# librosa/librosa

Hardware: AMD Instinct MI355X
Metric: STFT+mel frames/sec (n_fft=2048 hop=512) (higher is better)
Workload: dtype f32

## Files before the change

librosa_amd/csrc/lra_api.hip:

```cpp
#include <dlfcn.h>
#include <hip/hip_runtime.h>
#include <rocfft/rocfft.h>

#include <algorithm>
#include <atomic>
#include <chrono>
#include <cmath>
#include <cstdio>
#include <cstdlib>
#include <cstring>
#include <map>
#include <memory>
#include <mutex>
#include <string>
#include <thread>
#include <vector>

#include "../../include/librosa_amd.h"
#define LRA_FUSED_EXTERN
#include "lra_fused.h"
#include "lra_mel.h"
#include "lra_post.h"
#include "lra_pcen.h"
#include "lra_onset.h"
#include "lra_cqt.h"
#include "lra_hpss.h"
#include "lra_probe.h"
#include "lra_rng.h"
#include "lra_mixed_launch.h"
#include "lra_rhythm_launch.h"
#include "lra_beat_launch.h"
#include "lra_peaks_launch.h"
#include "lra_chroma_launch.h"

using namespace lra;

static thread_local std::string g_err;

static int fail(int code, const std::string& msg) {
    g_err = msg;
    return code;
}
#define LRA_HIP(expr)                                                                                        \
    do {                                                                                                     \
        hipError_t e__ = (expr);                                                                             \
        if (e__ != hipSuccess) return fail(LRA_EHIP, std::string(#expr) + ": " + hipGetErrorString(e__));    \
    } while (0)
#define LRA_FFT(expr)                                                                                        \
    do {                                                                                                     \
        rocfft_status s__ = (expr);                                                                          \
        if (s__ != rocfft_status_success) return fail(LRA_EROCFFT, std::string(#expr) + ": rocfft status " + std::to_string((int)s__)); \
    } while (0)
#define LRA_TRY(expr)              \
    do {                           \
        int rc__ = (expr);         \
        if (rc__ != LRA_OK) return rc__; \
    } while (0)

struct lra_ctx {
    int device = 0;
    hipStream_t own_stream = nullptr;
    hipStream_t stream = nullptr;
    int n_cu = 256;
    int opt_stft_iters = 0;
    int opt_istft_strip_groups = 0;
    int opt_variant = -1;
    int opt_autotune = 1;
    int opt_mel_runs = 1;
    int opt_mel_tile = 0;
    int opt_generic_mel = 0;
    int opt_lds_pad = 0;
    int opt_v2 = 1;
    int opt_istft16 = 0;
    int opt_placement_retry = 0;
    struct PlacedAlloc {
        size_t padded = 0;
        std::vector<hipMemGenericAllocationHandle_t> handles;
        bool plain = false;
    };
    std::map<void*, PlacedAlloc> placed;
    std::mutex placed_mu;
    std::vector<std::pair<void*, size_t>> placed_retired;
    size_t placed_va_spent = 0;
    static constexpr size_t kPlacedVaBudget = (size_t)4 << 40;
    double placed_best_gbps = 0.0;
    int opt_v3 = 1;
    int opt_mel_pc = 1;
    int opt_mel_many = 1;
    int opt_cqt_merge = 1;
    int opt_hpss_tile = 1;
    int opt_mixed_inv_pow2 = 1;
    int opt_mixed_pow2_mel = 1;
    int opt_ola4 = 1;
    int opt_mixed_irfft = 1;
    int opt_mixed = 1;
    int opt_direct = 1;
    int opt_xcd_remap = 1;
    unsigned int* d_flag = nullptr;
    std::map<std::pair<int, int>, std::pair<void*, void*>> cqt_tw;
    std::string name;
    struct HostPipe* pipe = nullptr;
    hipStream_t side_stream = nullptr;
    hipStream_t side_main = nullptr;
    static constexpr int kForkRing = 16;
    hipEvent_t fork_event[kForkRing] = {}, side_passed[kForkRing] = {};
    bool fork_used[kForkRing] = {};
    int fork_next = 0;
    static constexpr int kJoinRing = 8;
    hipEvent_t join_event[kJoinRing] = {}, main_passed[kJoinRing] = {};
    bool join_used[kJoinRing] = {};
    int join_next = 0;
    bool on_side = false, side_used = false;
    struct ResampleFft* rs_fft = nullptr;
    int opt_pipe_chunk_mb = 128;
    int opt_pipe_threads = 8;
};

// ... 146 lines not shown
    int* d_melr_addr = nullptr;
    int melr_zero = 0, melr_mid = 0, melr_pmax = 0;
    bool melr_ok = false;
    bool melr_many = false;
    void* d_melr2_w = nullptr;
    void* d_melr2_keep = nullptr;
    int* d_melr2_addr = nullptr;
    int melr2_zero = 0, melr2_mid = 0, melr2_pmax = 0;
    bool melr2_ok = false;
    int* d_run[2] = {nullptr, nullptr};
    int* d_segd[2] = {nullptr, nullptr};
    int nyq[2] = {0, 0};
    int n_pieces[2] = {0, 0};
};

struct lra_istft_plan {
    lra_ctx* ctx = nullptr;
    int n_fft = 0, hop = 0, center = 0, dtype = 0;
    bool pow2 = false;
    int logm = 0;
    void* d_win_scaled = nullptr;
    void* d_tw[kNumVariants] = {};
    int tuned_variant[4] = {-1, -1, -1, -1};
    void* d_twr = nullptr;
    FftPlanCache fft;
    Scratch spec, frames;
    Scratch norm;
    void* d_mtw = nullptr;
    void* d_mtwn = nullptr;
};

namespace {

static int resident_workgroups(const void* kern, int block, int lds) {
    static std::mutex mu;
    static std::map<std::pair<const void*, int>, int> cache;
    std::lock_guard<std::mutex> lk(mu);
    const auto key = std::make_pair(kern, lds);
    auto it = cache.find(key);
    if (it != cache.end()) return it->second;
    int per_cu = 0;
    if (lds > 65536) (void)hipFuncSetAttribute(kern, hipFuncAttributeMaxDynamicSharedMemorySize, lds);
    if (hipOccupancyMaxActiveBlocksPerMultiprocessor(&per_cu, kern, block, lds) != hipSuccess) per_cu = 0;
    (void)hipGetLastError();
    cache[key] = per_cu;
    return per_cu;
}

template <class T> struct StftLaunch {
    StftArgs<T> a;
    int mode = 0;
    long long batch = 0;
    int iters_opt = 0;
    int mel_tile_opt = 0;
    int n_cu = 256;
    void* out = nullptr;
    int lds_pad = 0;
    bool xcd_remap = true;
    bool use_v2 = true;
    bool use_direct = true;
    bool mel_v2 = false;
    bool mel_pc = false;
    bool mel_runs = true;
    const lra_mel_plan* mel = nullptr;
    hipStream_t stream = nullptr;
    hipError_t err = hipSuccess;

    template <class Cfg, int MODE> void launch(int shared_bytes) {
        static_assert(Cfg::P <= 4, "at most four Stockham passes are wired up");
        const int lds_probe_v1 = Cfg::FPB * stft_slot_bytes<Cfg>(MODE, a.n_mels, mel_tile_opt > 0 ? mel_tile_opt : 4) + shared_bytes + lds_pad;
        void (*kern)(StftArgs<T>, const T*, void*) = nullptr;
        bool direct = false;
        if constexpr (Cfg::PLAN == 0) {
        kern = stft_kernel<Cfg, MODE, POW_TWO, 0>;
        if (MODE != OUT_COMPLEX && a.power_mode == POW_ONE) kern = stft_kernel<Cfg, MODE, POW_ONE, 0>;
        if (MODE != OUT_COMPLEX && a.power_mode == POW_GENERAL) kern = stft_kernel<Cfg, MODE, POW_GENERAL, 0>;
        if constexpr (sizeof(T) == 4) {
            if (ring_rows_aligned<Cfg>(a.hop)) {
                kern = stft_kernel<Cfg, MODE, POW_TWO, 1>;
                if (MODE != OUT_COMPLEX && a.power_mode == POW_ONE) kern = stft_kernel<Cfg, MODE, POW_ONE, 1>;
                if (MODE != OUT_COMPLEX && a.power_mode == POW_GENERAL) kern = stft_kernel<Cfg, MODE, POW_GENERAL, 1>;
            }
        }
        if constexpr (MODE == OUT_COMPLEX || MODE == OUT_POWER) {
            if (a.hop >= Cfg::N && use_direct) {
                direct = true;
                kern = stft_kernel<Cfg, MODE, POW_TWO, 2>;
                if (MODE != OUT_COMPLEX && a.power_mode == POW_ONE) kern = stft_kernel<Cfg, MODE, POW_ONE, 2>;
                if (MODE != OUT_COMPLEX && a.power_mode == POW_GENERAL) kern = stft_kernel<Cfg, MODE, POW_GENERAL, 2>;
            }
        }
        if constexpr ((MODE == OUT_COMPLEX || MODE == OUT_POWER) && sizeof(T) == 4 && (Cfg::LOGM >= 12 || Cfg::LOGM == 7 || Cfg::LOGM == 8)) {
            const int hd = use_direct ? regring_hd<Cfg>(a.hop) : 0;
#define LRA_PICKR(RAM)                                                                                       \
    kern = stft_kernel<Cfg, MODE, POW_TWO, RAM>;                                                            \
    if (MODE != OUT_COMPLEX && a.power_mode == POW_ONE) kern = stft_kernel<Cfg, MODE, POW_ONE, RAM>;        \
    if (MODE != OUT_COMPLEX && a.power_mode == POW_GENERAL) kern = stft_kernel<Cfg, MODE, POW_GENERAL, RAM>;
            if (hd == 2) { direct = true; LRA_PICKR(3) } else if (hd == 4) { direct = true; LRA_PICKR(4) } else if (hd == 8) { direct = true; LRA_PICKR(5) } else if (hd == 16) { direct = true; LRA_PICKR(6) }
#undef LRA_PICKR
        }
        }
        bool v2 = false;
        if constexpr (v23_cfg_ok<Cfg>() && (MODE == OUT_COMPLEX || MODE == OUT_POWER || MODE == OUT_MELR)) {
            const int hd = (use_v2 && (MODE != OUT_MELR || mel_v2)) ? v2_hop_divisor<Cfg>(a.hop) : 0;
            if (hd) {
                v2 = true;
// ... 11 lines not shown
        if (iters <= 0) {
            const int per_cu = lds_probe <= 160 * 1024 ? resident_workgroups(reinterpret_cast<const void*>(kern), Cfg::NT, lds_probe) : 0;
            const long long conc = (long long)n_cu * (per_cu > 0 ? per_cu : 1);
            const int fpb = Cfg::FPB;
            int best_iters = 0;
            double best_fill = -1.0;
            for (int cand = 176; cand >= 24; --cand) {
                const int wgpc = (a.n_frames + fpb * cand - 1) / (fpb * cand);
                const int it = (a.n_frames + fpb * wgpc - 1) / (fpb * wgpc);
                const double rounds = (double)(batch * wgpc) / (double)conc;
                const double fill = (v2 && Cfg::TF == 64 && rounds <= 1.0 && rounds >= 0.6) ? 1.0 : rounds / std::ceil(rounds);
                if (fill > best_fill + 0.02) { best_fill = fill; best_iters = it; }
            }
            iters = best_iters;
            while (iters > 4 && batch * ((a.n_frames + fpb * iters - 1) / (fpb * iters)) < 2LL * n_cu) iters /= 2;
        }
        if (iters < 1) iters = 1;
        a.rot_uniform = 0;
        if (Cfg::FPB > 1 && Cfg::TF < 64 && ring_rows_aligned<Cfg>(a.hop)) {
            if (iters_opt <= 0 && iters >= 4) iters = (iters + 3) / 4 * 4;
            a.rot_uniform = iters % 4 == 0;
        }
        a.mel_tile = mel_tile_opt > 0 ? mel_tile_opt : 4;
        if (a.mel_tile > iters) a.mel_tile = iters;
        a.frames_per_wg = Cfg::FPB * iters;
        a.wg_per_clip = (a.n_frames + a.frames_per_wg - 1) / a.frames_per_wg;
        a.slot_bytes = v2 ? stft2_slot_bytes<Cfg>() : direct ? Cfg::FRAME_BYTES : stft_slot_bytes<Cfg>(MODE, a.n_mels, a.mel_tile);
        a.shared_off = Cfg::FPB * a.slot_bytes;
        const long long grid = batch * a.wg_per_clip;
        if (grid > 0x7ffffff0LL) { err = hipErrorInvalidConfiguration; return; }
        const int lds = Cfg::FPB * a.slot_bytes + shared_bytes + lds_pad;
        if (lds > 160 * 1024) { err = hipErrorInvalidValue; return; }
        if (lds > 65536) {
            err = hipFuncSetAttribute(reinterpret_cast<const void*>(kern), hipFuncAttributeMaxDynamicSharedMemorySize, lds);
            if (err != hipSuccess) return;
        }
        a.n_blocks = (int)grid;
        a.xcd_chunk = (xcd_remap && grid >= 64) ? (int)((grid + 7) / 8) : 0;
        const long long launch_grid = a.xcd_chunk ? 8LL * a.xcd_chunk : grid;
        hipLaunchKernelGGL(kern, dim3((unsigned)launch_grid), dim3(Cfg::NT), lds, stream, a, a.y, out);
        err = hipGetLastError();
    }

    template <class Cfg> void launch_pc(int hd) {
        using PL = PcLayout<Cfg>;
        void (*kern)(StftArgs<T>, const T*, void*) = nullptr;
#define LRA_PICKP(HD)                                                        \
    kern = stft_pc_kernel<Cfg, HD, POW_TWO>;                                 \
    if (a.power_mode == POW_ONE) kern = stft_pc_kernel<Cfg, HD, POW_ONE>;    \
    if (a.power_mode == POW_GENERAL) kern = stft_pc_kernel<Cfg, HD, POW_GENERAL>;
        if (hd == 4) { LRA_PICKP(4) } else { LRA_PICKP(8) }
#undef LRA_PICKP
        const int lds = PL::BYTES + lds_pad;
        constexpr int fpb = PL::NP;
        int iters = iters_opt;
        if (iters <= 0) {
            const int per_cu = resident_workgroups(reinterpret_cast<const void*>(kern), PL::NT, lds);
            const long long conc = (long long)n_cu * (per_cu > 0 ? per_cu : 1);
            int best_iters = 0;
            double best_fill = -1.0;
            for (int cand = 176; cand >= 24; --cand) {
                const int wgpc = (a.n_frames + fpb * cand - 1) / (fpb * cand);
                const int it = (a.n_frames + fpb * wgpc - 1) / (fpb * wgpc);
                const double rounds = (double)(batch * wgpc) / (double)conc;
                const double fill = (rounds <= 1.0 && rounds >= 0.6) ? 1.0 : rounds / std::ceil(rounds);
                if (fill > best_fill + 0.02) { best_fill = fill; best_iters = it; }
            }
            iters = best_iters;
            while (iters > 4 && batch * ((a.n_frames + fpb * iters - 1) / (fpb * iters)) < 2LL * n_cu) iters /= 2;
        }
        if (iters < 1) iters = 1;
        a.rot_uniform = 0;
        a.mel_tile = 1;
        a.frames_per_wg = fpb * iters;
        a.wg_per_clip = (a.n_frames + a.frames_per_wg - 1) / a.frames_per_wg;
        a.slot_bytes = PL::FRAME;
        a.shared_off = 0;
        const long long grid = batch * a.wg_per_clip;
        if (grid > 0x7ffffff0LL) { err = hipErrorInvalidConfiguration; return; }
        a.n_blocks = (int)grid;
        a.xcd_chunk = (xcd_remap && grid >= 64) ? (int)((grid + 7) / 8) : 0;
        const long long launch_grid = a.xcd_chunk ? 8LL * a.xcd_chunk : grid;
        hipLaunchKernelGGL(kern, dim3((unsigned)launch_grid), dim3(PL::NT), lds, stream, a, a.y, out);
        err = hipGetLastError();
    }

    template <class Cfg> void operator()() {
        if constexpr (Cfg::REV) {
            err = hipErrorInvalidValue;
            return;
        } else if constexpr (Cfg::PLAN == 1) {
            if (!use_v2 || v2_hop_divisor<Cfg>(a.hop) == 0) { err = hipErrorInvalidValue; return; }
            if (mode == OUT_COMPLEX) launch<Cfg, OUT_COMPLEX>(0);
            else if (mode == OUT_POWER) launch<Cfg, OUT_POWER>(0);
            else if (mode == OUT_MEL2 && mel_pc && mel && mel->melr2_ok && mel_runs) {
                if constexpr (pc_cfg_ok<Cfg>()) {
                    const int hd_pc = v2_hop_divisor<Cfg>(a.hop);
                    if (!pc_bank_ok<Cfg>(a.n_mels, mel->melr2_pmax) || !pc_fits_budget<Cfg>(hd_pc, a.power_mode)) { err = hipErrorInvalidValue; return; }
                    a.melr_w = (const T*)mel->d_melr2_w;
                    a.melr_keep = (const T*)mel->d_melr2_keep;
                    a.melr_addr = mel->d_melr2_addr;
                    a.melr_zero = mel->melr2_zero;
                    a.melr_mid = mel->melr2_mid;
                    a.melr_pmax = mel->melr2_pmax;
                    launch_pc<Cfg>(hd_pc);
                } else err = hipErrorInvalidValue;
            } else err = hipErrorInvalidValue;
        } else {
            run<Cfg>();
        }
    }
    template <class Cfg> void run() {
        if (mode == OUT_MEL2) {
            using MC = typename MelCfgOf<Cfg>::type;
            if constexpr (pc_cfg_ok<Cfg>()) {
                const int hd_pc = v2_hop_divisor<Cfg>(a.hop);
                if (mel_pc && mel && mel->melr2_ok && mel_runs && use_v2 && pc_bank_ok<Cfg>(a.n_mels, mel->melr2_pmax) && pc_fits_budget<Cfg>(hd_pc, a.power_mode)) {
                    a.melr_w = (const T*)mel->d_melr2_w;
                    a.melr_keep = (const T*)mel->d_melr2_keep;
                    a.melr_addr = mel->d_melr2_addr;
                    a.melr_zero = mel->melr2_zero;
                    a.melr_mid = mel->melr2_mid;
                    a.melr_pmax = mel->melr2_pmax;
                    launch_pc<Cfg>(hd_pc);
                    return;
                }
            }
            if constexpr (v2_cfg_ok<MC>()) {
                if (mel && mel->melr2_ok && mel_runs && use_v2 && melr_fits<MC>() && v2_hop_divisor<MC>(a.hop) > 0) {
                    const int shared_r = melr_shared_bytes<MC>(a.n_mels, mel->melr2_pmax);
                    if (MC::FPB * stft2_slot_bytes<MC>() + shared_r <= 160 * 1024) {
                        a.melr_w = (const T*)mel->d_melr2_w;
                        a.melr_keep = (const T*)mel->d_melr2_keep;
                        a.melr_addr = mel->d_melr2_addr;
                        a.melr_zero = mel->melr2_zero;
// ... 492 lines not shown
}

template <class T>
int stft_run(lra_stft_plan* p, int mode, const void* y, int64_t batch, int64_t n, int64_t y_stride, double power, lra_mel_plan* mel, void* out, int64_t row_pitch = 0) {
    LRA_BIND(p->ctx);
    int64_t n_frames = 0;
    LRA_TRY(lra_stft_num_frames(p, n, &n_frames));
    if (batch <= 0) return LRA_OK;
    if (!y || !out) return fail(LRA_EINVAL, "null data pointer");
    if (y_stride < n) return fail(LRA_EINVAL, "y_stride smaller than n");
    if (n_frames > 0x7fffffffLL / 4) return fail(LRA_EINVAL, "too many frames per clip");
    lra_ctx* ctx = p->ctx;
    const int bins = p->n_fft / 2 + 1;
    if (row_pitch <= 0) row_pitch = bins;
    if (row_pitch != bins && (!p->pow2 || row_pitch < bins || (mode != OUT_COMPLEX && mode != OUT_POWER)))
        return fail(LRA_EINVAL, "a row pitch other than n_bins is served by the fused power-of-two kernels only (complex / power results), and must be at least n_bins");
    if (mode == OUT_MEL) {
        if (!mel) return fail(LRA_EINVAL, "null mel plan");
        if (mel->n_bins != bins) return fail(LRA_EINVAL, "mel basis has " + std::to_string(mel->n_bins) + " bins, stft has " + std::to_string(bins));
        if (mel->dtype != p->dtype) return fail(LRA_EINVAL, "mel plan dtype differs from stft plan dtype");
    }
    const bool pow2_mel_mixed = p->pow2 && mode == OUT_MEL && p->d_mtw && ctx->opt_mixed && ctx->opt_mixed_pow2_mel && row_pitch == bins && mel &&
                                mel->n_mels >= (p->n_fft >= 256 ? 56 : 40);
    if (p->pow2 && !pow2_mel_mixed) {
        StftLaunch<T> L;
        L.a = StftArgs<T>();
        L.a.y = (const T*)y;
        L.a.y_stride = y_stride;
        L.a.n = n;
        L.a.n_frames = (int)n_frames;
        L.a.row_pitch = row_pitch;
        L.a.hop = p->hop;
        L.a.pad = p->center ? p->n_fft / 2 : 0;
        L.a.pad_mode = p->pad_mode;
        L.a.win = (const T*)p->d_win;
        L.a.twr = (const cx<T>*)p->d_twr;
        L.out = out;
        L.a.power_mode = power_mode_of(power);
        L.a.power = (T)power;
        if (mel) {
            L.a.mel_c0 = mel->d_c0;
            L.a.mel_len = mel->d_len;
            L.a.mel_off = mel->d_off;
            L.a.mel_val = (const T*)mel->d_val;
            L.a.n_mels = mel->n_mels;
            L.a.mel_wAB = (const T*)mel->d_wAB;
            L.mel = mel;
        }
        L.a.nonfinite_flag = ctx->d_flag;
        L.mode = (mode == OUT_MEL && mel && mel->two_slope && !ctx->opt_generic_mel) ? OUT_MEL2 : mode;
        L.batch = batch;
        L.stream = ctx->stream;
        L.iters_opt = ctx->opt_stft_iters;
        L.n_cu = ctx->n_cu;
        L.mel_tile_opt = ctx->opt_mel_tile;
        L.lds_pad = ctx->opt_lds_pad;
        L.xcd_remap = ctx->opt_xcd_remap != 0;
        L.use_v2 = ctx->opt_v2 != 0;
        L.mel_pc = ctx->opt_mel_pc != 0;
        L.use_direct = ctx->opt_direct != 0;
        L.mel_runs = ctx->opt_mel_runs != 0;
        int variant = ctx->opt_variant >= 0 ? ctx->opt_variant : 0;
        auto launch = [&](int v) -> int {
            StftLaunch<T> Lv = L;
            Lv.a.tw = (const cx<T>*)p->d_tw[v];
            if (!dispatch_logm<T>(p->logm, v, Lv)) return fail(LRA_EINVAL, "unsupported power-of-two size");
            if (Lv.err != hipSuccess) return fail(LRA_EHIP, std::string("stft kernel launch: ") + hipGetErrorString(Lv.err));
            return LRA_OK;
        };
        bool v2_applies = false;
        if constexpr (sizeof(T) == 4)
            v2_applies = ctx->opt_v2 && (L.mode == OUT_COMPLEX || L.mode == OUT_POWER) && p->logm == 10 && v2_hop_divisor<typename CfgSel<float, 10, 0>::type>(p->hop) > 0;
        if (ctx->opt_variant < 0 && ctx->opt_autotune && sizeof(T) == 4 && p->logm == 10 && !v2_applies) {
            int& tuned = p->tuned_variant[L.mode & 3];
            if (tuned < 0 && batch * n_frames >= 65536) LRA_TRY(autotune_variant(ctx, launch, &tuned));
            if (tuned >= 0) variant = tuned;
        }
        bool pc_g = false;
        if constexpr (sizeof(T) == 4) {
            using C6 = typename CfgSel<float, 10, 6>::type;
            if (L.mode == OUT_MEL2 && ctx->opt_mel_pc == 2 && p->logm == 10 && mel && mel->melr2_ok && ctx->opt_mel_runs && ctx->opt_v2 && (ctx->opt_variant < 0 || ctx->opt_variant == 6))
                pc_g = pc_bank_ok<C6>(mel->n_mels, mel->melr2_pmax) && pc_fits_budget<C6>(v2_hop_divisor<C6>(p->hop), power_mode_of(power));
        }
        if ((v2_applies && (ctx->opt_v3 == 2 || (ctx->opt_v3 == 1 && L.mode == OUT_COMPLEX)) && (ctx->opt_variant < 0 || ctx->opt_variant == 6)) || pc_g) variant = 6;
        else if (variant == 6) variant = 0;
        return launch(variant);
    }
    if (p->d_mtw && ctx->opt_mixed) {
        mixed::Args<T> a = mixed::Args<T>();
        a.y = (const T*)y;
        a.y_stride = y_stride;
        a.n = n;
        a.n_frames = (int)n_frames;
        a.hop = p->hop;
        a.pad = p->center ? p->n_fft / 2 : 0;
        a.pad_mode = p->pad_mode;
        a.win = (const T*)(p->pow2 ? p->d_win_full : p->d_win);
        a.tw_m = (const mixed::cpx<T>*)p->d_mtw;
        a.tw_n = (const mixed::cpx<T>*)p->d_mtwn;
        a.power_mode = power_mode_of(power);
        a.power = (T)power;
        const int F = mixed::frames_per_group_of(p->n_fft, (int)sizeof(T));
        a.groups_per_clip = (int)((n_frames + F - 1) / F);
        int mm = mixed::MIXED_COMPLEX;
        if (mode == OUT_COMPLEX) {
            a.D = (mixed::cpx<T>*)out;
// ... 607 lines not shown
                LRA_HIP(hipStreamCreateWithFlags(&ctx->side_stream, hipStreamNonBlocking));
        }
        const int slot = ctx->fork_next;
        ctx->fork_next = (slot + 1) % lra_ctx::kForkRing;
        if (!ctx->fork_event[slot]) LRA_HIP(hipEventCreateWithFlags(&ctx->fork_event[slot], hipEventDisableTiming));
        if (!ctx->side_passed[slot]) LRA_HIP(hipEventCreateWithFlags(&ctx->side_passed[slot], hipEventDisableTiming));
        if (ctx->fork_used[slot]) LRA_HIP(hipEventSynchronize(ctx->side_passed[slot]));
        LRA_HIP(hipEventRecord(ctx->fork_event[slot], ctx->stream));
        LRA_HIP(hipStreamWaitEvent(ctx->side_stream, ctx->fork_event[slot], 0));
        LRA_HIP(hipEventRecord(ctx->side_passed[slot], ctx->side_stream));
        ctx->fork_used[slot] = true;
        ctx->side_main = ctx->stream;
        ctx->stream = ctx->side_stream;
        ctx->on_side = ctx->side_used = true;
        return LRA_OK;
    }
    if (mode == LRA_SIDE_BACK) {
        if (!ctx->on_side) return fail(LRA_EINVAL, "lra_ctx_side: not on the side stream");
        ctx->stream = ctx->side_main;
        ctx->on_side = false;
        return LRA_OK;
    }
    if (mode == LRA_SIDE_END && ctx->on_side) {
        ctx->stream = ctx->side_main;
        ctx->on_side = false;
    }
    if (mode == LRA_SIDE_JOIN || mode == LRA_SIDE_END) {
        if (ctx->on_side) return fail(LRA_EINVAL, "lra_ctx_side: join from the main stream (LRA_SIDE_BACK first)");
        if (!ctx->side_used) return LRA_OK;
        const int js = ctx->join_next;
        ctx->join_next = (js + 1) % lra_ctx::kJoinRing;
        if (!ctx->join_event[js]) LRA_HIP(hipEventCreateWithFlags(&ctx->join_event[js], hipEventDisableTiming));
        if (!ctx->main_passed[js]) LRA_HIP(hipEventCreateWithFlags(&ctx->main_passed[js], hipEventDisableTiming));
        if (ctx->join_used[js]) LRA_HIP(hipEventSynchronize(ctx->main_passed[js]));
        LRA_HIP(hipEventRecord(ctx->join_event[js], ctx->side_stream));
        LRA_HIP(hipStreamWaitEvent(ctx->stream, ctx->join_event[js], 0));
        LRA_HIP(hipEventRecord(ctx->main_passed[js], ctx->stream));
        ctx->join_used[js] = true;
        ctx->side_used = false;
        return LRA_OK;
    }
    return fail(LRA_EINVAL, "lra_ctx_side: mode must be LRA_SIDE_FORK, LRA_SIDE_BACK, LRA_SIDE_JOIN or LRA_SIDE_END");
}

int lra_ctx_sync(lra_ctx* ctx) {
    LRA_BIND(ctx);
    LRA_HIP(hipStreamSynchronize(ctx->stream));
    return LRA_OK;
}

int lra_ctx_set_option(lra_ctx* ctx, const char* key, int value) {
    if (!ctx || !key) return fail(LRA_EINVAL, "null argument");
    if (!std::strcmp(key, "stft_iters")) ctx->opt_stft_iters = value;
    else if (!std::strcmp(key, "istft_strip_groups")) ctx->opt_istft_strip_groups = value;
    else if (!std::strcmp(key, "mel_tile")) ctx->opt_mel_tile = value;
    else if (!std::strcmp(key, "ablate")) (void)value;
    else if (!std::strcmp(key, "generic_mel")) ctx->opt_generic_mel = value;
    else if (!std::strcmp(key, "pipe_chunk_mb")) ctx->opt_pipe_chunk_mb = value > 0 ? value : 128;
    else if (!std::strcmp(key, "pipe_threads")) ctx->opt_pipe_threads = value > 0 ? value : 1;
    else if (!std::strcmp(key, "lds_pad")) ctx->opt_lds_pad = value;
    else if (!std::strcmp(key, "xcd_remap")) ctx->opt_xcd_remap = value != 0;
    else if (!std::strcmp(key, "v2")) ctx->opt_v2 = value != 0;
    else if (!std::strcmp(key, "mel_pc")) ctx->opt_mel_pc = (value == 1 || value == 2) ? value : 0;
    else if (!std::strcmp(key, "istft16")) ctx->opt_istft16 = value != 0;
    else if (!std::strcmp(key, "placement_retry")) ctx->opt_placement_retry = value < 0 ? 0 : (value > 8 ? 8 : value);
    else if (!std::strcmp(key, "v3")) ctx->opt_v3 = (value == 1 || value == 2) ? value : 0;
    else if (!std::strcmp(key, "cqt_merge")) ctx->opt_cqt_merge = value < 0 ? 0 : (value > 2 ? 2 : (int)value);
    else if (!std::strcmp(key, "mel_many")) ctx->opt_mel_many = value != 0;
    else if (!std::strcmp(key, "direct")) ctx->opt_direct = value != 0;
    else if (!std::strcmp(key, "mixed")) ctx->opt_mixed = value == 2 ? 2 : (value != 0);
    else if (!std::strcmp(key, "hpss_tile")) ctx->opt_hpss_tile = value != 0;
    else if (!std::strcmp(key, "mixed_pow2_mel")) ctx->opt_mixed_pow2_mel = value != 0;
    else if (!std::strcmp(key, "ola4")) ctx->opt_ola4 = value != 0;
    else if (!std::strcmp(key, "mixed_irfft")) ctx->opt_mixed_irfft = value != 0;
    else if (!std::strcmp(key, "mixed_inv_pow2")) ctx->opt_mixed_inv_pow2 = value != 0;
    else if (!std::strcmp(key, "autotune")) ctx->opt_autotune = value != 0;
    else if (!std::strcmp(key, "mel_runs")) ctx->opt_mel_runs = value != 0;
    else if (!std::strcmp(key, "variant")) ctx->opt_variant = (value >= 0 && value < kNumVariants) ? value : -1;
    else return fail(LRA_EINVAL, std::string("unknown option ") + key);
    return LRA_OK;
}

int lra_ctx_nonfinite_reset(lra_ctx* ctx) {
    LRA_BIND(ctx);
    LRA_HIP(hipMemsetAsync(ctx->d_flag, 0, sizeof(unsigned int), ctx->stream));
    return LRA_OK;
}

int lra_ctx_nonfinite_read(lra_ctx* ctx, int* flag) {
    LRA_BIND(ctx);
    if (!flag) return fail(LRA_EINVAL, "null flag");
    unsigned int h = 0;
    LRA_HIP(hipMemcpyAsync(&h, ctx->d_flag, sizeof(h), hipMemcpyDeviceToHost, ctx->stream));
    LRA_HIP(hipStreamSynchronize(ctx->stream));
    if (h & 2u) {
        (void)hipMemsetAsync(ctx->d_flag, 0, sizeof(unsigned int), ctx->stream);
        return fail(LRA_EHIP, "fused mel kernel: a producer / consumer hand-over timed out (results invalid); ctx option mel_pc = 0 selects the one-wave kernel");
    }
    *flag = (int)(h & 1u);
    return LRA_OK;
}

int lra_ctx_device_name(lra_ctx* ctx, char* buf, size_t buflen) {
    if (!ctx || !buf || !buflen) return fail(LRA_EINVAL, "null argument");
    std::snprintf(buf, buflen, "%s, %d CUs", ctx->name.c_str(), ctx->n_cu);
    return LRA_OK;
// ... 1855 lines not shown
```

librosa_amd/csrc/lra_fused.h:

```cpp
#pragma once

#include <hip/hip_runtime.h>

#include "lra_dispatch.h"
#include "lra_kernels_pc.h"

template <class Cfg, int MODE, int PM, int RA>
__global__ __launch_bounds__(Cfg::NT, Cfg::MIN_WAVES) void stft_kernel(lra::StftArgs<typename Cfg::real> a, const typename Cfg::real* __restrict__ y,
                                                                     void* __restrict__ out) {
    extern __shared__ __attribute__((aligned(16))) char lra_smem[];
    lra::Lds lds;
    lds.base = lra_smem;
    a.y = y;
    a.D = static_cast<typename Cfg::cplx*>(out);
    a.S = static_cast<typename Cfg::real*>(out);
    a.Mel = static_cast<typename Cfg::real*>(out);
    const int blk = lra::xcd_block((int)blockIdx.x, a.xcd_chunk);
    if (blk >= a.n_blocks) return;
    lra::stft_block<Cfg, MODE, PM, RA>(a, blk, lds);
}

constexpr int kV3Waves = 3;
template <class Cfg, int HD, int MODE, int PM>
__global__ __launch_bounds__(Cfg::NT, (Cfg::NT > 256 ? 1 : (Cfg::TF == 64 && HD >= 4 && PM != lra::POW_GENERAL && MODE != lra::OUT_MELR ? (Cfg::PLAN == 1 ? kV3Waves : 3) : 2))) void stft2_kernel(lra::StftArgs<typename Cfg::real> a, const typename Cfg::real* __restrict__ y,
                                                                                  void* __restrict__ out) {
    extern __shared__ __attribute__((aligned(16))) char lra_smem[];
    lra::Lds lds;
    lds.base = lra_smem;
    a.y = y;
    a.D = static_cast<typename Cfg::cplx*>(out);
    a.S = static_cast<typename Cfg::real*>(out);
    a.Mel = static_cast<typename Cfg::real*>(out);
    const int blk = lra::xcd_block((int)blockIdx.x, a.xcd_chunk);
    if (blk >= a.n_blocks) return;
    lra::stft_block2<Cfg, HD, MODE, PM>(a, blk, lds);
}

template <class Cfg, int HD, int PM>
__global__ __launch_bounds__(lra::PcLayout<Cfg>::NT, 3) void stft_pc_kernel(lra::StftArgs<typename Cfg::real> a, const typename Cfg::real* __restrict__ y, void* __restrict__ out) {
    extern __shared__ __attribute__((aligned(32))) char lra_smem[];
    lra::Lds lds;
    lds.base = lra_smem;
    a.y = y;
    a.Mel = static_cast<typename Cfg::real*>(out);
    const int blk = lra::xcd_block((int)blockIdx.x, a.xcd_chunk);
    if (blk >= a.n_blocks) return;
    lra::stft_pc_block<Cfg, HD, PM>(a, blk, lds);
}

template <class Cfg, int HC>
__global__ __launch_bounds__(Cfg::NT, Cfg::MIN_WAVES) void istft_kernel(lra::IstftArgs<typename Cfg::real> a, const typename Cfg::cplx* __restrict__ D,
                                                                      const typename Cfg::real* __restrict__ wss, typename Cfg::real* __restrict__ y) {
    extern __shared__ __attribute__((aligned(16))) char lra_smem[];
    lra::Lds lds;
    lds.base = lra_smem;
    a.D = D;
    a.wss = wss;
    a.y = y;
    const int blk = lra::xcd_block((int)blockIdx.x, a.xcd_chunk);
    if (blk >= a.n_blocks) return;
    lra::istft_block<Cfg, HC>(a, blk, lds);
}


namespace lra {

#define LRA_CFG_ALIAS(NAME, ...) using NAME = typename CfgSel<__VA_ARGS__>::type; using NAME##_mel = typename MelCfgOf<NAME>::type; using NAME##_melmany = typename MelManyCfgOf<NAME>::type;
LRA_CFG_ALIAS(cfg_f32_4, float, 4, 0)
LRA_CFG_ALIAS(cfg_f32_5, float, 5, 0)
LRA_CFG_ALIAS(cfg_f32_6, float, 6, 0)
LRA_CFG_ALIAS(cfg_f32_7, float, 7, 0)
LRA_CFG_ALIAS(cfg_f32_8, float, 8, 0)
LRA_CFG_ALIAS(cfg_f32_9, float, 9, 0)
LRA_CFG_ALIAS(cfg_f32_10, float, 10, 0)
LRA_CFG_ALIAS(cfg_f32_10v1, float, 10, 1)
LRA_CFG_ALIAS(cfg_f32_10v4, float, 10, 4)
LRA_CFG_ALIAS(cfg_f32_10r, float, 10, 5)
LRA_CFG_ALIAS(cfg_f32_10g, float, 10, 6)
LRA_CFG_ALIAS(cfg_f32_10q, float, 10, 7)
LRA_CFG_ALIAS(cfg_f32_11, float, 11, 0)
LRA_CFG_ALIAS(cfg_f32_12, float, 12, 0)
LRA_CFG_ALIAS(cfg_f32_13, float, 13, 0)
LRA_CFG_ALIAS(cfg_f64_4, double, 4, 0)
LRA_CFG_ALIAS(cfg_f64_5, double, 5, 0)
LRA_CFG_ALIAS(cfg_f64_6, double, 6, 0)
LRA_CFG_ALIAS(cfg_f64_7, double, 7, 0)
LRA_CFG_ALIAS(cfg_f64_8, double, 8, 0)
LRA_CFG_ALIAS(cfg_f64_9, double, 9, 0)
LRA_CFG_ALIAS(cfg_f64_10, double, 10, 0)
LRA_CFG_ALIAS(cfg_f64_11, double, 11, 0)
LRA_CFG_ALIAS(cfg_f64_12, double, 12, 0)
#undef LRA_CFG_ALIAS

}

#define LRA_STFT_SET(S, C, RA)                                                                       \
    S(lra::C, 0, 2, RA)                                                                              \
    S(lra::C, 1, 1, RA) S(lra::C, 1, 2, RA) S(lra::C, 1, 3, RA)                                      \
    S(lra::C, 2, 1, RA) S(lra::C, 2, 2, RA) S(lra::C, 2, 3, RA)                                      \
    S(lra::C##_mel, 3, 1, RA) S(lra::C##_mel, 3, 2, RA) S(lra::C##_mel, 3, 3, RA)                   \
// ... 54 lines not shown
```

librosa_amd/csrc/lra_kernels_pc.h:

```cpp
#pragma once

#include "lra_kernels2.h"

namespace lra {

constexpr int kPcPrioPA = 3, kPcPrioPS = 2, kPcPrioCA = 0, kPcPrioCB = 1;
constexpr int kPcSpinLimit = 1 << 22;

template <class Cfg> struct PcLayout {
    using T = typename Cfg::real;
    static constexpr int NP = 2;
    static constexpr int NT = (NP + 1) * Cfg::TF;
    static constexpr int FRAME = Cfg::FRAME_BYTES;
    static constexpr int PW = (v2_pw_bytes<Cfg>() + 15) / 16 * 16;
    static constexpr int RS = ((Cfg::R * (Cfg::TF + kMelRsPitchExtra) + 2) * 2 * (int)sizeof(T) + 15) / 16 * 16;
    static constexpr int frame_off(int s) { return s * FRAME; }
    static constexpr int pw_off(int s) { return NP * FRAME + s * PW; }
    static constexpr int rs_off() { return NP * (FRAME + PW); }
    static constexpr int flags_off() { return rs_off() + RS; }
    static constexpr int ready_off(int s) { return flags_off() + 4 * s; }
    static constexpr int consumed_off(int s) { return flags_off() + 4 * (NP + s); }
    static constexpr int BYTES = flags_off() + 16;
};

// ... 206 lines not shown
        lds_st<C>(rs, a.melr_zero, mk<T>((T)0, (T)0));
    }
}
template <class Cfg, int S, bool UNI> LRA_HD PcTileV pc_combine(const StftArgs<typename Cfg::real>& a, int clip, int frame, int tf, int it, bool last_of_slot, PcRegs<Cfg>& rg, Lds wg, PcTileV mt) {
    using T = typename Cfg::real;
    using RG = PcRegs<Cfg>;
    constexpr int PH = RG::PH, NB = RG::NB, MT = RG::TILE;
    T x[NB][2 * PH];
    LRA_UNROLL
    for (int b = 0; b < NB; ++b) {
        LRA_UNROLL
        for (int q = 0; q < 2 * PH; ++q) {
            const cx<T> pr = pc_pair_ld(wg, rg.mad[b][q]);
            x[b][q] = q < PH ? pr.y : pr.x;
        }
    }
    LRA_UNROLL
    for (int b = 0; b < NB; ++b) {
        const int m = NB * tf + b;
        if (m >= a.n_mels) break;
        T part[2];
        LRA_UNROLL
        for (int h = 0; h < 2; ++h) {
            T acc = (T)0;
            LRA_UNROLL
            for (int q = 0; q < PH; ++q) acc += x[b][h * PH + q];
            part[h] = acc;
        }
        const T v = part[0] + part[1];
        int s8;
        if constexpr (UNI) {
            s8 = (rg.ph[S][b] + it) & (MT - 1);
            mt[MT * b + s8] = v;
        } else {
            s8 = (int)((rg.row[b] - a.Mel + frame) & (MT - 1));
            LRA_UNROLL
            for (int k = 0; k < MT; ++k) mt[MT * b + k] = k == s8 ? v : mt[MT * b + k];
        }
        if (last_of_slot || s8 == MT - 1) {
            T t8[MT];
            pc_tile_band(mt, b, t8);
            melr_burst_row(rg.row[b] + (frame - s8), s8, it, t8);
        }
    }
    return mt;
}

#ifndef LRA_HOSTSIM
template <class Cfg, bool UNI> __device__ __forceinline__ void pc_consumer(const StftArgs<typename Cfg::real>& a, int clip, int f_first, int iters, int n_it, Lds lds) {
    using L = PcLayout<Cfg>;
    constexpr int TF = Cfg::TF;
    PcRegs<Cfg> rg;
    const Lds rs = lds_sub(lds, L::rs_off());
    const int tf = (int)(threadIdx.x & (TF - 1));
    pc_consumer_prologue<Cfg>(a, clip, f_first, iters, tf, rg, lds);
    pc_fence();
    for (int it = 0; it < n_it; ++it) {
#define LRA_PC_SERVE(S)                                                                                                        \
        {                                                                                                                      \
            const int frame = f_first + S * iters + it;                                                                       \
            v2_setprio<kPcPrioCA>();                                                                                      \
            pc_wait_ready(lds, L::ready_off(S), it + 1, a.nonfinite_flag);                                                     \
            pc_runs_read<Cfg>(rg, lds_sub(lds, L::pw_off(S)));                                                                 \
            pc_fence();                                                                                                        \
            if (tf == 0) pc_flag_store(lds, L::consumed_off(S), it + 1);                             \
            pc_fence();                                                                                                        \
            pc_accumulate<Cfg>(a, tf, rg, rs);                                                                                 \
            pc_fence();                                                                                                        \
            v2_setprio<kPcPrioCB>();                                                                                      \
            if (frame < a.n_frames) rg.mt[S] = pc_combine<Cfg, S, UNI>(a, clip, frame, tf, it, it + 1 == iters || frame + 1 >= a.n_frames, rg, lds, rg.mt[S]); \
            pc_fence();                                                                                                        \
        }
        LRA_PC_SERVE(0)
        LRA_PC_SERVE(1)
#undef LRA_PC_SERVE
    }
}
#endif

template <class Cfg, int HD, int PM = POW_TWO> LRA_HD void stft_pc_block(const StftArgs<typename Cfg::real>& a_in, const int blk, Lds lds) {
    static_assert(pc_cfg_ok<Cfg>(), "producer / consumer mel kernel: one wave per frame, mirrored last pass, swizzled power row");
    using T = typename Cfg::real;
    using L = PcLayout<Cfg>;
    using RG = Regs2<Cfg, HD>;
    constexpr int NP = L::NP, TF = Cfg::TF;
    StftArgs<T> a = a_in;
    const int clip = blk / a.wg_per_clip;
    const int f_first = (blk % a.wg_per_clip) * a.frames_per_wg;
    const int iters = a.frames_per_wg / NP;
    const int left = a.n_frames - f_first;
    const int n_it = left < iters ? left : iters;
#ifdef LRA_HOSTSIM
    LRA_REGS(RG, prg, L::NT);
    LRA_REGS(PcRegs<Cfg>, crg, L::NT);
    LRA_PHASE(L::NT, tid) {
        const int w = tid / TF, tf = tid % TF;
        if (w < NP) pc_producer_prologue<Cfg, HD>(a, clip, f_first + w * iters, tf, LRA_R(prg));
        else pc_consumer_prologue<Cfg>(a, clip, f_first, iters, tf, LRA_R(crg), lds);
        if (tid < 2 * NP) pc_flag_store(lds, L::flags_off() + 4 * tid, 0);
    } LRA_PHASE_END
    for (int it = 0; it < n_it; ++it) {
        LRA_PHASE(L::NT, tid) {
            const int w = tid / TF, tf = tid % TF;
            if (w < NP) pc_producer_pass0<Cfg, HD>(a, clip, f_first + w * iters + it, it, it + 1 < iters, tf, LRA_R(prg), lds_sub(lds, L::frame_off(w)));
        } LRA_PHASE_END_SYNC(true)
#define LRA_PC_MID(p)                                                                                                                   \
        if (Cfg::P - 1 > p) {                                                                                                           \
            LRA_PHASE(L::NT, tid) {                                                                                                     \
                if (tid / TF < NP) pass_read<Cfg, (p < Cfg::P ? p : 0)>(LRA_R(prg).v, lds_sub(lds, L::frame_off(tid / TF)), tid % TF);  \
            } LRA_PHASE_END_SYNC(true)                                                                                                  \
            LRA_PHASE(L::NT, tid) {                                                                                                     \
                if (tid / TF < NP) pc_mid_dft_write<Cfg, (p < Cfg::P ? p : 0)>(LRA_R(prg).v, LRA_R(prg).treg, lds_sub(lds, L::frame_off(tid / TF)), tid % TF); \
            } LRA_PHASE_END_SYNC(true)                                                                                                  \
        }
        LRA_PC_MID(1)
        LRA_PC_MID(2)
#undef LRA_PC_MID
        LRA_PHASE(L::NT, tid) {
            if (tid / TF < NP) pc_last_read<Cfg, HD>(LRA_R(prg), lds_sub(lds, L::frame_off(tid / TF)), tid % TF);
        } LRA_PHASE_END_SYNC(true)
        LRA_PHASE(L::NT, tid) {
            const int w = tid / TF, tf = tid % TF, frame = f_first + w * iters + it;
            if (w < NP) pc_last_power_row<Cfg, HD, PM>(a, clip, frame, tf, LRA_R(prg), lds_sub(lds, L::pw_off(w)));
        } LRA_PHASE_END
        for (int s = 0; s < NP; ++s) {
            LRA_PHASE(L::NT, tid) {
                if (tid / TF == NP) pc_runs_read<Cfg>(LRA_R(crg), lds_sub(lds, L::pw_off(s)));
            } LRA_PHASE_END_SYNC(true)
            LRA_PHASE(L::NT, tid) {
                if (tid / TF == NP) pc_accumulate<Cfg>(a, tid % TF, LRA_R(crg), lds_sub(lds, L::rs_off()));
            } LRA_PHASE_END_SYNC(true)
            LRA_PHASE(L::NT, tid) {
                const int tf = tid % TF, frame = f_first + s * iters + it;
                if (tid / TF == NP && frame < a.n_frames) {
                    const bool last = it + 1 == iters || frame + 1 >= a.n_frames;
                    if (pc_tile_uniform<Cfg>(a)) {
                        if (s == 0) LRA_R(crg).mt[0] = pc_combine<Cfg, 0, true>(a, clip, frame, tf, it, last, LRA_R(crg), lds, LRA_R(crg).mt[0]);
                        else LRA_R(crg).mt[1] = pc_combine<Cfg, 1, true>(a, clip, frame, tf, it, last, LRA_R(crg), lds, LRA_R(crg).mt[1]);
                    } else {
                        if (s == 0) LRA_R(crg).mt[0] = pc_combine<Cfg, 0, false>(a, clip, frame, tf, it, last, LRA_R(crg), lds, LRA_R(crg).mt[0]);
                        else LRA_R(crg).mt[1] = pc_combine<Cfg, 1, false>(a, clip, frame, tf, it, last, LRA_R(crg), lds, LRA_R(crg).mt[1]);
                    }
                }
            } LRA_PHASE_END_SYNC(true)
        }
        sim::state().barrier();
    }
#else
    static_assert((TF & (TF - 1)) == 0 && L::pw_off(0) % 32 == 0 && L::PW % 32 == 0, "lane mask; power rows start on 32 bytes (v2_pw_addr_xor)");
    if (threadIdx.x < 2 * NP) pc_flag_store(lds, L::flags_off() + 4 * (int)threadIdx.x, 0);
    phase_sync<false>();
    const int wave = LRA_UNIFORM((int)(threadIdx.x / TF));
    if (wave < NP) {
        RG rg;
        const Lds fr = lds_sub(lds, L::frame_off(wave)), pwr = lds_sub(lds, L::pw_off(wave));
        {
            const int tf = (phase_tid() & (TF - 1));
            pc_producer_prologue<Cfg, HD>(a, clip, f_first + wave * iters, tf, rg);
        }
        pc_fence();
        for (int it = 0; it < n_it; ++it) {
            const int frame = f_first + wave * iters + it;
            v2_setprio<kPcPrioPA>();
            {
                const int tf = (phase_tid() & (TF - 1));
                pc_producer_pass0<Cfg, HD>(a, clip, frame, it, it + 1 < iters, tf, rg, fr);
            }
            pc_fence();
#define LRA_PC_MID(p)                                                                                    \
            if (Cfg::P - 1 > p) {                                                                        \
                { const int tf = (phase_tid() & (TF - 1)); pass_read<Cfg, (p < Cfg::P ? p : 0)>(rg.v, fr, tf); } \
                pc_fence();                                                                              \
                { const int tf = (phase_tid() & (TF - 1)); pc_mid_dft_write<Cfg, (p < Cfg::P ? p : 0)>(rg.v, rg.treg, fr, tf); } \
                pc_fence();                                                                              \
            }
            LRA_PC_MID(1)
            LRA_PC_MID(2)
#undef LRA_PC_MID
            int taken;
            {
                const int tf = (phase_tid() & (TF - 1));
                pc_last_read<Cfg, HD>(rg, fr, tf);
                taken = pc_flag_load(lds, L::consumed_off(wave));
            }
            pc_fence();
            v2_setprio<kPcPrioPS>();
            if (LRA_UNLIKELY(LRA_UNIFORM(taken) < it)) pc_wait(lds, L::consumed_off(wave), it, a.nonfinite_flag);
            {
                const int tf = (phase_tid() & (TF - 1));
                pc_last_power_row<Cfg, HD, PM>(a, clip, frame, tf, rg, pwr);
            }
            pc_fence();
            if ((phase_tid() & (TF - 1)) == 0) pc_flag_store(lds, L::ready_off(wave), it + 1);
            pc_fence();
        }
    } else {
        if (pc_tile_uniform<Cfg>(a)) pc_consumer<Cfg, true>(a, clip, f_first, iters, n_it, lds);
        else pc_consumer<Cfg, false>(a, clip, f_first, iters, n_it, lds);
    }
#endif
}

}
```

Before: 647.9 million.

## Make producer-consumer STFT kernel persistent with cost-model grid geometry

Converts the producer/consumer STFT kernel into a persistent grid. The grid is capped at the number of resident workgroups, and each workgroup walks several work items, re-reading its kernel arguments from the kernarg segment. Strip length is now picked by a cost model (items per workgroup times iters plus a fixed per-item cost) instead of a wave-fill heuristic. This is meant to cut tail effects and launch imbalance, at the price of an extra barrier between items and a more complex XCD remap for padded grids.

```diff
diff --git a/librosa_amd/csrc/lra_api.hip b/librosa_amd/csrc/lra_api.hip
--- a/librosa_amd/csrc/lra_api.hip
+++ b/librosa_amd/csrc/lra_api.hip
@@ -28,6 +28,7 @@
 #include "lra_probe.h"
 #include "lra_rng.h"
 #include "lra_mixed_launch.h"
+#include "lra_pc_geom.h"
 #include "lra_rhythm_launch.h"
 #include "lra_beat_launch.h"
 #include "lra_peaks_launch.h"
@@ -63,6 +64,7 @@
     hipStream_t stream = nullptr;
     int n_cu = 256;
     int opt_stft_iters = 0;
+    int opt_pc_grid = 0;
     int opt_istft_strip_groups = 0;
     int opt_variant = -1;
     int opt_autotune = 1;
@@ -315,6 +317,7 @@
     int mode = 0;
     long long batch = 0;
     int iters_opt = 0;
+    int pc_grid_opt = 0;
     int mel_tile_opt = 0;
     int n_cu = 256;
     void* out = nullptr;
@@ -432,35 +435,27 @@
         if (hd == 4) { LRA_PICKP(4) } else { LRA_PICKP(8) }
 #undef LRA_PICKP
         const int lds = PL::BYTES + lds_pad;
-        constexpr int fpb = PL::NP;
-        int iters = iters_opt;
-        if (iters <= 0) {
-            const int per_cu = resident_workgroups(reinterpret_cast<const void*>(kern), PL::NT, lds);
-            const long long conc = (long long)n_cu * (per_cu > 0 ? per_cu : 1);
-            int best_iters = 0;
-            double best_fill = -1.0;
-            for (int cand = 176; cand >= 24; --cand) {
-                const int wgpc = (a.n_frames + fpb * cand - 1) / (fpb * cand);
-                const int it = (a.n_frames + fpb * wgpc - 1) / (fpb * wgpc);
-                const double rounds = (double)(batch * wgpc) / (double)conc;
-                const double fill = (rounds <= 1.0 && rounds >= 0.6) ? 1.0 : rounds / std::ceil(rounds);
-                if (fill > best_fill + 0.02) { best_fill = fill; best_iters = it; }
-            }
-            iters = best_iters;
-            while (iters > 4 && batch * ((a.n_frames + fpb * iters - 1) / (fpb * iters)) < 2LL * n_cu) iters /= 2;
-        }
-        if (iters < 1) iters = 1;
+        const int per_cu = resident_workgroups(reinterpret_cast<const void*>(kern), PL::NT, lds);
+        const long long resident = (long long)n_cu * (per_cu > 0 ? per_cu : 1);
+        const PcGeom g = pc_geometry(batch, a.n_frames, PL::NP, resident, iters_opt, pc_grid_opt);
         a.rot_uniform = 0;
         a.mel_tile = 1;
-        a.frames_per_wg = fpb * iters;
-        a.wg_per_clip = (a.n_frames + a.frames_per_wg - 1) / a.frames_per_wg;
+        a.frames_per_wg = PL::NP * g.iters;
+        a.wg_per_clip = g.wg_per_clip;
         a.slot_bytes = PL::FRAME;
         a.shared_off = 0;
-        const long long grid = batch * a.wg_per_clip;
-        if (grid > 0x7ffffff0LL) { err = hipErrorInvalidConfiguration; return; }
-        a.n_blocks = (int)grid;
-        a.xcd_chunk = (xcd_remap && grid >= 64) ? (int)((grid + 7) / 8) : 0;
-        const long long launch_grid = a.xcd_chunk ? 8LL * a.xcd_chunk : grid;
+        if (g.items + g.grid + 8 > 0x7ffffff0LL) { err = hipErrorInvalidConfiguration; return; }
+        a.n_blocks = (int)g.items;
+        long long launch_grid = g.grid;
+        a.xcd_chunk = 0;
+        if (xcd_remap && g.items >= 64) {
+            const long long chunk = (g.items + 7) / 8;
+            const long long padded_grid = 8 * chunk <= g.grid + 7 && g.items <= g.grid ? 8 * chunk : g.grid / 8 * 8;
+            if (padded_grid >= 8) {
+                a.xcd_chunk = (int)chunk;
+                launch_grid = padded_grid;
+            }
+        }
         hipLaunchKernelGGL(kern, dim3((unsigned)launch_grid), dim3(PL::NT), lds, stream, a, a.y, out);
         err = hipGetLastError();
     }
@@ -1059,6 +1054,7 @@
         L.batch = batch;
         L.stream = ctx->stream;
         L.iters_opt = ctx->opt_stft_iters;
+        L.pc_grid_opt = ctx->opt_pc_grid;
         L.n_cu = ctx->n_cu;
         L.mel_tile_opt = ctx->opt_mel_tile;
         L.lds_pad = ctx->opt_lds_pad;
@@ -1772,6 +1768,7 @@
 int lra_ctx_set_option(lra_ctx* ctx, const char* key, int value) {
     if (!ctx || !key) return fail(LRA_EINVAL, "null argument");
     if (!std::strcmp(key, "stft_iters")) ctx->opt_stft_iters = value;
+    else if (!std::strcmp(key, "pc_grid")) ctx->opt_pc_grid = value > 0 ? value : 0;
     else if (!std::strcmp(key, "istft_strip_groups")) ctx->opt_istft_strip_groups = value;
     else if (!std::strcmp(key, "mel_tile")) ctx->opt_mel_tile = value;
     else if (!std::strcmp(key, "ablate")) (void)value;
diff --git a/librosa_amd/csrc/lra_fused.h b/librosa_amd/csrc/lra_fused.h
--- a/librosa_amd/csrc/lra_fused.h
+++ b/librosa_amd/csrc/lra_fused.h
@@ -36,16 +36,44 @@
     lra::stft_block2<Cfg, HD, MODE, PM>(a, blk, lds);
 }
 
+namespace lra {
+template <class T> struct PcKernArgs {
+    StftArgs<T> a;
+    const T* y;
+    void* out;
+};
+template <class Cfg, int HD, int PM, bool PRODUCER>
+__device__ __forceinline__ void stft_pc_item(StftArgs<typename Cfg::real> a, const typename Cfg::real* __restrict__ y, void* __restrict__ out, int blk, int wave, Lds lds) {
+    a.y = y;
+    a.Mel = static_cast<typename Cfg::real*>(out);
+    pc_role_item<Cfg, HD, PM, PRODUCER>(a, blk, wave, lds);
+}
+template <class Cfg, int HD, int PM, bool PRODUCER> __device__ __forceinline__ void stft_pc_walk(int wave, Lds lds) {
+    using KA = PcKernArgs<typename Cfg::real>;
+    auto kp = __builtin_amdgcn_kernarg_segment_ptr();
+    int item = (int)blockIdx.x;
+    while (true) {
+        asm volatile("" : "+s"(kp));
+        const KA* __restrict__ ka = (const KA*)kp;
+        const int chunk = ka->a.xcd_chunk;
+        if (chunk > 0 && (item >> 3) >= chunk) return;
+        const int blk = xcd_block(item, chunk);
+        if (blk >= ka->a.n_blocks) return;
+        if (item != (int)blockIdx.x) phase_sync<false>();
+        stft_pc_item<Cfg, HD, PM, PRODUCER>(ka->a, ka->y, ka->out, blk, wave, lds);
+        item += (int)gridDim.x;
+    }
+}
+}
 template <class Cfg, int HD, int PM>
-__global__ __launch_bounds__(lra::PcLayout<Cfg>::NT, 3) void stft_pc_kernel(lra::StftArgs<typename Cfg::real> a, const typename Cfg::real* __restrict__ y, void* __restrict__ out) {
+__global__ __launch_bounds__(lra::PcLayout<Cfg>::NT, 3) void stft_pc_kernel(lra::StftArgs<typename Cfg::real>, const typename Cfg::real* __restrict__, void* __restrict__) {
+    static_assert(alignof(lra::StftArgs<typename Cfg::real>) == 8 && sizeof(lra::StftArgs<typename Cfg::real>) % 8 == 0, "PcKernArgs mirrors the argument block");
     extern __shared__ __attribute__((aligned(32))) char lra_smem[];
     lra::Lds lds;
     lds.base = lra_smem;
-    a.y = y;
-    a.Mel = static_cast<typename Cfg::real*>(out);
-    const int blk = lra::xcd_block((int)blockIdx.x, a.xcd_chunk);
-    if (blk >= a.n_blocks) return;
-    lra::stft_pc_block<Cfg, HD, PM>(a, blk, lds);
+    const int wave = LRA_UNIFORM((int)(threadIdx.x / Cfg::TF));
+    if (wave < lra::PcLayout<Cfg>::NP) lra::stft_pc_walk<Cfg, HD, PM, true>(wave, lds);
+    else lra::stft_pc_walk<Cfg, HD, PM, false>(wave, lds);
 }
 
 template <class Cfg, int HC>
diff --git a/librosa_amd/csrc/lra_kernels_pc.h b/librosa_amd/csrc/lra_kernels_pc.h
--- a/librosa_amd/csrc/lra_kernels_pc.h
+++ b/librosa_amd/csrc/lra_kernels_pc.h
@@ -282,7 +282,7 @@
     constexpr int TF = Cfg::TF;
     PcRegs<Cfg> rg;
     const Lds rs = lds_sub(lds, L::rs_off());
-    const int tf = (int)(threadIdx.x & (TF - 1));
+    const int tf = (phase_tid() & (TF - 1));
     pc_consumer_prologue<Cfg>(a, clip, f_first, iters, tf, rg, lds);
     pc_fence();
     for (int it = 0; it < n_it; ++it) {
@@ -305,6 +305,71 @@
         LRA_PC_SERVE(1)
 #undef LRA_PC_SERVE
     }
+}
+template <class Cfg, int HD, int PM> __device__ __forceinline__ void pc_producer_item(const StftArgs<typename Cfg::real>& a, int clip, int f_first, int iters, int n_it, int wave, Lds lds) {
+    using L = PcLayout<Cfg>;
+    using RG = Regs2<Cfg, HD>;
+    constexpr int TF = Cfg::TF;
+    static_assert((TF & (TF - 1)) == 0 && L::pw_off(0) % 32 == 0 && L::PW % 32 == 0, "lane mask; power rows start on 32 bytes (v2_pw_addr_xor)");
+    RG rg;
+    const Lds fr = lds_sub(lds, L::frame_off(wave)), pwr = lds_sub(lds, L::pw_off(wave));
+    {
+        const int tf = (phase_tid() & (TF - 1));
+        pc_producer_prologue<Cfg, HD>(a, clip, f_first + wave * iters, tf, rg);
+    }
+    pc_fence();
+    for (int it = 0; it < n_it; ++it) {
+        const int frame = f_first + wave * iters + it;
+        v2_setprio<kPcPrioPA>();
+        {
+            const int tf = (phase_tid() & (TF - 1));
+            pc_producer_pass0<Cfg, HD>(a, clip, frame, it, it + 1 < iters, tf, rg, fr);
+        }
+        pc_fence();
+#define LRA_PC_MID(p)                                                                                    \
+        if (Cfg::P - 1 > p) {                                                                        \
+            { const int tf = (phase_tid() & (TF - 1)); pass_read<Cfg, (p < Cfg::P ? p : 0)>(rg.v, fr, tf); } \
+            pc_fence();                                                                              \
+            { const int tf = (phase_tid() & (TF - 1)); pc_mid_dft_write<Cfg, (p < Cfg::P ? p : 0)>(rg.v, rg.treg, fr, tf); } \
+            pc_fence();                                                                              \
+        }
+        LRA_PC_MID(1)
+        LRA_PC_MID(2)
+#undef LRA_PC_MID
+        int taken;
+        {
+            const int tf = (phase_tid() & (TF - 1));
+            pc_last_read<Cfg, HD>(rg, fr, tf);
+            taken = pc_flag_load(lds, L::consumed_off(wave));
+        }
+        pc_fence();
+        v2_setprio<kPcPrioPS>();
+        if (LRA_UNLIKELY(LRA_UNIFORM(taken) < it)) pc_wait(lds, L::consumed_off(wave), it, a.nonfinite_flag);
+        {
+            const int tf = (phase_tid() & (TF - 1));
+            pc_last_power_row<Cfg, HD, PM>(a, clip, frame, tf, rg, pwr);
+        }
+        pc_fence();
+        if ((phase_tid() & (TF - 1)) == 0) pc_flag_store(lds, L::ready_off(wave), it + 1);
+        pc_fence();
+    }
+}
+template <class Cfg, int HD, int PM, bool PRODUCER> __device__ __forceinline__ void pc_role_item(const StftArgs<typename Cfg::real>& a, int blk, int wave, Lds lds) {
+    using L = PcLayout<Cfg>;
+    constexpr int NP = L::NP;
+    const int clip = blk / a.wg_per_clip;
+    const int f_first = (blk % a.wg_per_clip) * a.frames_per_wg;
+    const int iters = a.frames_per_wg / NP;
+    const int left = a.n_frames - f_first;
+    const int n_it = left < iters ? left : iters;
+    if constexpr (PRODUCER) {
+        const int t = phase_tid();
+        if (t < 2 * NP) pc_flag_store(lds, L::flags_off() + 4 * t, 0);
+    }
+    phase_sync<false>();
+    if constexpr (PRODUCER) pc_producer_item<Cfg, HD, PM>(a, clip, f_first, iters, n_it, wave, lds);
+    else if (pc_tile_uniform<Cfg>(a)) pc_consumer<Cfg, true>(a, clip, f_first, iters, n_it, lds);
+    else pc_consumer<Cfg, false>(a, clip, f_first, iters, n_it, lds);
 }
 #endif
 
@@ -377,57 +442,9 @@
         sim::state().barrier();
     }
 #else
-    static_assert((TF & (TF - 1)) == 0 && L::pw_off(0) % 32 == 0 && L::PW % 32 == 0, "lane mask; power rows start on 32 bytes (v2_pw_addr_xor)");
-    if (threadIdx.x < 2 * NP) pc_flag_store(lds, L::flags_off() + 4 * (int)threadIdx.x, 0);
-    phase_sync<false>();
     const int wave = LRA_UNIFORM((int)(threadIdx.x / TF));
-    if (wave < NP) {
-        RG rg;
-        const Lds fr = lds_sub(lds, L::frame_off(wave)), pwr = lds_sub(lds, L::pw_off(wave));
-        {
-            const int tf = (phase_tid() & (TF - 1));
-            pc_producer_prologue<Cfg, HD>(a, clip, f_first + wave * iters, tf, rg);
-        }
-        pc_fence();
-        for (int it = 0; it < n_it; ++it) {
-            const int frame = f_first + wave * iters + it;
-            v2_setprio<kPcPrioPA>();
-            {
-                const int tf = (phase_tid() & (TF - 1));
-                pc_producer_pass0<Cfg, HD>(a, clip, frame, it, it + 1 < iters, tf, rg, fr);
-            }
-            pc_fence();
-#define LRA_PC_MID(p)                                                                                    \
-            if (Cfg::P - 1 > p) {                                                                        \
-                { const int tf = (phase_tid() & (TF - 1)); pass_read<Cfg, (p < Cfg::P ? p : 0)>(rg.v, fr, tf); } \
-                pc_fence();                                                                              \
-                { const int tf = (phase_tid() & (TF - 1)); pc_mid_dft_write<Cfg, (p < Cfg::P ? p : 0)>(rg.v, rg.treg, fr, tf); } \
-                pc_fence();                                                                              \
-            }
-            LRA_PC_MID(1)
-            LRA_PC_MID(2)
-#undef LRA_PC_MID
-            int taken;
-            {
-                const int tf = (phase_tid() & (TF - 1));
-                pc_last_read<Cfg, HD>(rg, fr, tf);
-                taken = pc_flag_load(lds, L::consumed_off(wave));
-            }
-            pc_fence();
-            v2_setprio<kPcPrioPS>();
-            if (LRA_UNLIKELY(LRA_UNIFORM(taken) < it)) pc_wait(lds, L::consumed_off(wave), it, a.nonfinite_flag);
-            {
-                const int tf = (phase_tid() & (TF - 1));
-                pc_last_power_row<Cfg, HD, PM>(a, clip, frame, tf, rg, pwr);
-            }
-            pc_fence();
-            if ((phase_tid() & (TF - 1)) == 0) pc_flag_store(lds, L::ready_off(wave), it + 1);
-            pc_fence();
-        }
-    } else {
-        if (pc_tile_uniform<Cfg>(a)) pc_consumer<Cfg, true>(a, clip, f_first, iters, n_it, lds);
-        else pc_consumer<Cfg, false>(a, clip, f_first, iters, n_it, lds);
-    }
+    if (wave < NP) pc_role_item<Cfg, HD, PM, true>(a, blk, wave, lds);
+    else pc_role_item<Cfg, HD, PM, false>(a, blk, wave, lds);
 #endif
 }
 
diff --git a/librosa_amd/csrc/lra_pc_geom.h b/librosa_amd/csrc/lra_pc_geom.h
--- /dev/null
+++ b/librosa_amd/csrc/lra_pc_geom.h
@@ -0,0 +1,53 @@
+#pragma once
+
+namespace lra {
+
+constexpr int kPcItemCost = 3;
+constexpr int kPcMinStrip = 24;
+
+struct PcGeom {
+    int iters = 1;
+    int wg_per_clip = 1;
+    long long items = 0;
+    long long grid = 0;
+    long long items_per_wg = 0;
+};
+
+inline long long pc_ceil_div(long long a, long long b) { return (a + b - 1) / b; }
+
+inline PcGeom pc_geom_for(long long batch, int n_frames, int np, long long resident, int iters) {
+    PcGeom g;
+    g.iters = iters < 1 ? 1 : iters;
+    g.wg_per_clip = (int)pc_ceil_div(n_frames, (long long)np * g.iters);
+    if (g.wg_per_clip < 1) g.wg_per_clip = 1;
+    g.items = batch * g.wg_per_clip;
+    g.grid = g.items < resident ? g.items : resident;
+    if (g.grid < 1) g.grid = 1;
+    g.items_per_wg = pc_ceil_div(g.items, g.grid);
+    return g;
+}
+
+inline PcGeom pc_geometry(long long batch, int n_frames, int np, long long resident, int iters_opt = 0, long long grid_cap = 0) {
+    if (batch < 1) batch = 1;
+    if (n_frames < 1) n_frames = 1;
+    if (np < 1) np = 1;
+    if (resident < 1) resident = 1;
+    if (grid_cap > 0 && grid_cap < resident) resident = grid_cap;
+    if (iters_opt > 0) {
+        return pc_geom_for(batch, n_frames, np, resident, iters_opt);
+    }
+    const int max_wgpc = n_frames / (np * kPcMinStrip) > 1 ? n_frames / (np * kPcMinStrip) : 1;
+    PcGeom best;
+    long long best_cost = -1;
+    int last_iters = 0;
+    for (int wgpc = 1; wgpc <= max_wgpc; ++wgpc) {
+        const PcGeom g = pc_geom_for(batch, n_frames, np, resident, (int)pc_ceil_div(n_frames, (long long)np * wgpc));
+        if (g.iters == last_iters) continue;
+        last_iters = g.iters;
+        const long long cost = g.items_per_wg * (g.iters + kPcItemCost);
+        if (best_cost < 0 || cost < best_cost) { best = g; best_cost = cost; }
+    }
+    return best;
+}
+
+}
```

Measured after the change: 645.2 million. About the same (-0.4%).
